# graphdeco-inria/reduced-3dgs

Measured on AMD Instinct MI355X. Metric: train iters/s (fwd+bwd) + Mpix/s render, 500k Gaussians @1600x1062, higher is better.
Workload: dtype f32

## Files before the change

reduced-3dgs_amd/csrc/binning.hip:

```cpp
#include <cstdlib>
#include <cstring>
#include <mutex>
#include <string>

#include <rocprim/rocprim.hpp>

#include "depth_sort.h"

namespace r3 {

struct GatherTiles {
    const uint32_t* tiles;
    __host__ __device__ uint32_t operator()(uint32_t id) const { return tiles[id]; }
};

size_t depth_sort_temp_bytes(size_t P)
{
    size_t a = 0, b = 0;
    uint32_t* n = nullptr;
    R3_HIP(rocprim::radix_sort_pairs(nullptr, a, n, n, rocprim::counting_iterator<uint32_t>(0), n, P, 0, 32));
    auto it = rocprim::make_transform_iterator(n, GatherTiles{n});
    R3_HIP(rocprim::inclusive_scan(nullptr, b, it, n, P, rocprim::plus<uint32_t>()));
    return (a > b ? a : b) + 256;
}

void run_generic_depth_sort(int P, GeomState& g, hipStream_t s)
{
    size_t bytes = g.temp_bytes;
    R3_HIP(rocprim::radix_sort_pairs(g.temp, bytes, g.depth_key, g.key_sorted, rocprim::counting_iterator<uint32_t>(0),
                                     g.order, (size_t)P, 0, 32, s));
    bytes = g.temp_bytes;
    auto it = rocprim::make_transform_iterator(g.order, GatherTiles{g.tiles});
    R3_HIP(rocprim::inclusive_scan(g.temp, bytes, it, g.offsets, (size_t)P, rocprim::plus<uint32_t>(), s));
}

__global__ __launch_bounds__(1024) void header_reduce_kernel(const HeaderArgs* __restrict__ ap)
{
    __shared__ uint32_t s_red[16][6];
    const HeaderArgs a = *ap;
    const PrePartial all = reduce_partials(a.parts, a.n_parts, s_red);
    if (threadIdx.x == 0) write_header(a, all);
}

void issue_header_reduce(const HeaderArgs* a, hipStream_t s)
{
    hipLaunchKernelGGL(header_reduce_kernel, dim3(1), dim3(1024), 0, s, a);
}

PairLayout pair_layout(int P, size_t n_tiles)
{
    static const int forced = [] {
        const char* v = getenv("R3DGS_TILE_SORT");
        return !v ? 0 : std::string(v) == "wide" ? 1 : std::string(v) == "split" ? 2 : 0;
    }();
    PairLayout l;
    l.tile_bits = (int)higher_msb((uint32_t)n_tiles);
    const int rb = (int)higher_msb((uint32_t)P);
    const bool fits16 = n_tiles <= 65536;
    if (forced == 1 || (forced == 2 && !fits16))
        l.wide = 1;
    else if (forced == 2)
        l.wide = 2;
    else
        l.wide = l.tile_bits + rb > 32 ? (fits16 ? 2 : 1) : 0;
// ... 94 lines not shown
        }
        if (lane == 0) {
            s_j[w] = j;
            if (w == 0) s_start0 = j == 0 ? 0u : offsets[j - 1];
        }
    }
    __syncthreads();
    const uint32_t j_lo = s_j[0], j_hi = s_j[1];
    const uint32_t n = min(j_hi - j_lo + 1u, (uint32_t)kEmitSlice);
    const uint32_t start0 = s_start0;
    auto stage = [&](uint32_t r0, uint32_t nr) {
        for (uint32_t k = threadIdx.x; k < nr; k += 256) {
            const uint32_t g = j_lo + r0 + k, id = a.order[g];
            s_start[k] = r0 + k == 0 ? start0 : offsets[g - 1];
            s_id[k] = id;
            s_rect[k] = a.rect_sorted ? a.rect_sorted[g] : a.rect[id];
        }
    };
    const uint32_t nr0 = min(n, (uint32_t)kEmitStage);
    stage(0u, nr0);
    __syncthreads();
    for (uint32_t k = threadIdx.x; k < n; k += 256) {
        const uint32_t start = k < nr0 ? s_start[k] : offsets[j_lo + k - 1];
        a.rec[k < nr0 ? s_id[k] : a.order[j_lo + k]].pair_start = start;
        if (start >= pos0) s_owner[start - pos0] = (unsigned short)k;
    }
    __syncthreads();
    {
        constexpr int E = kEmitPerBlock / 256;
        const int lane = threadIdx.x & 63, w = threadIdx.x >> 6;
        uint32_t v[E];
#pragma unroll
        for (int i = 0; i < E; i++) v[i] = s_owner[threadIdx.x * E + i];
#pragma unroll
        for (int i = 1; i < E; i++) v[i] = max(v[i], v[i - 1]);
        uint32_t incl = v[E - 1];
        for (int off = 1; off < 64; off <<= 1) {
            const uint32_t up = (uint32_t)__shfl_up((int)incl, off);
            if (lane >= off) incl = max(incl, up);
        }
        if (lane == 63) s_wmax[w] = incl;
        uint32_t before = (uint32_t)__shfl_up((int)incl, 1);
        if (lane == 0) before = 0;
        __syncthreads();
        for (int q = 0; q < w; q++) before = max(before, s_wmax[q]);
#pragma unroll
        for (int i = 0; i < E; i++) s_owner[threadIdx.x * E + i] = (unsigned short)max(v[i], before);
    }
    typedef typename IO::Reg Word;
    const int rank_bits = a.rank_bits;
    for (uint32_t r0 = 0; r0 < n; r0 += (uint32_t)kEmitStage) {
        const uint32_t nr = min(n - r0, (uint32_t)kEmitStage);
        __syncthreads();
        if (r0 > 0) {
            stage(r0, nr);
            __syncthreads();
        }
#pragma unroll
        for (int e = 0; e < kEmitPerBlock / 256; e++) {
            const uint32_t pos = pos0 + threadIdx.x + (uint32_t)e * 256u;
            if (pos < pos1) {
                const uint32_t lo = (uint32_t)s_owner[pos - pos0] - r0;
                if (lo < nr) {
                    const uint32_t local = pos - s_start[lo];
                    const ushort4 r = s_rect[lo];
                    const uint32_t w = (uint32_t)r.z - (uint32_t)r.x;
                    const uint32_t ty = local / w, tx = local - ty * w;
                    const uint32_t tile = ((uint32_t)r.y + ty) * (uint32_t)a.gx + (uint32_t)r.x + tx;
                    IO::store(a.words_out, nullptr, a.cap, pos, ((Word)tile << rank_bits) | (Word)s_id[lo]);
                    if (a.pair_rank) a.pair_rank[pos] = s_id[lo];
                    atomicAdd(&s_hist[tile & (uint32_t)(bins - 1)], 1u);
                }
            }
        }
    }
    __syncthreads();
    if ((int)threadIdx.x < bins) a.radix_rows[(size_t)threadIdx.x * a.row_stride + blk] = s_hist[threadIdx.x];
}

template <class IO>
__global__ __launch_bounds__(256) void emit_pairs_kernel(const EmitArgs* __restrict__ ap)
{
    const EmitArgs a = *ap;
    const uint32_t R = a.hdr->num_pairs;
    for (uint32_t t = blockIdx.x * 256u + threadIdx.x; t < a.n_tiles; t += gridDim.x * 256u) a.ranges[t] = make_uint2(0u, 0u);
    for (uint32_t blk = blockIdx.x; blk * (uint32_t)kEmitPerBlock < R; blk += gridDim.x) {
        emit_pairs_block<IO>(a, R, blk);
        __syncthreads();
    }
}

template <class IO>
__device__ __forceinline__ void radix_hist_block(const RadixArgs& a, uint32_t R, uint32_t blk)
// ... 300 lines not shown
```

reduced-3dgs_amd/csrc/blend.hip:

```cpp
#include <cstdlib>

#include "blend_math.h"
#include "common.h"

namespace r3 {

constexpr int kChunk = 64;

#if defined(R3_TIMELINE) || defined(R3_TIMELINE_FWD)
__device__ unsigned long long g_timeline[4 * 65536];
#define R3_TL_BEGIN_(id) const unsigned long long tl0_ = __builtin_amdgcn_s_memtime(); const uint32_t tlid_ = (id);
#define R3_TL_END_(extra)                                                                                                \
    if (threadIdx.x == 0 && tlid_ < 65536u) {                                                                            \
        g_timeline[4 * tlid_] = tl0_;                                                                                     \
        g_timeline[4 * tlid_ + 1] = __builtin_amdgcn_s_memtime();                                                         \
        g_timeline[4 * tlid_ + 2] = (unsigned long long)__builtin_amdgcn_s_getreg((4 << 0) | (0 << 6) | (31 << 11)) |     \
                                    ((unsigned long long)__builtin_amdgcn_s_getreg((20 << 0) | (0 << 6) | (31 << 11)) << 32); \
        g_timeline[4 * tlid_ + 3] = (unsigned long long)(extra);                                                          \
    }
#endif
#if defined(R3_TIMELINE)
#define R3_TL_BEGIN(id) R3_TL_BEGIN_(id)
#define R3_TL_END(extra) R3_TL_END_(extra)
#else
// ... 525 lines not shown
                }
            if (hit != 0ull) {
                const float z = wave_reduce9(sg, lane);
                int joff = j * kGradStride;
                asm("" : "+s"(joff));
                if (writer) s_grad_slot[joff] = z;
                contributed |= 1ull << j;
#ifndef R3_OLD_TRIP_FORMS
                {
                    typedef float v4f __attribute__((ext_vector_type(4)));
                    const volatile v4f __attribute__((address_space(3)))* zp =
                        (const volatile v4f __attribute__((address_space(3)))*)reinterpret_cast<float*>(s_zero);
                    const v4f z0 = zp[0], z1 = zp[1];
                    const float z2 = *(const volatile float __attribute__((address_space(3)))*)(zp + 2);
                    sg.sx = z0.x; sg.sy = z0.y; sg.sxx = z0.z; sg.sxy = z0.w;
                    sg.syy = z1.x; sg.sm = z1.y; sg.r = z1.z; sg.g = z1.w; sg.b = z2;
                }
#else
                sg.sx = sg.sy = sg.sxx = sg.sxy = sg.syy = sg.sm = sg.r = sg.g = sg.b = 0.f;
#endif
            }
        }
        __syncthreads();
        if (lane < n && ((contributed >> lane) & 1ull)) {
            const float4 c = s_rec[lane].c;
            const uint32_t rect_min = __float_as_uint(c.y), width = __float_as_uint(c.z) & 0xffffu;
            const uint32_t slot = __float_as_uint(c.w) + ((uint32_t)tile_y - (rect_min >> 16)) * width +
                                  ((uint32_t)tile_x - (rect_min & 0xffffu));
            float4* dst = reinterpret_cast<float4*>(a.pair_grad + (size_t)slot * kPairStride);
            const float* src = s_grad + lane * kGradStride;
            SplatSums u;
            u.sx = src[0];
            u.sy = src[1];
            u.sxx = src[2];
            u.sxy = src[3];
            u.syy = src[4];
            u.sm = src[5];
            u.r = src[6];
            u.g = src[7];
            u.b = src[8];
            const SplatGrad g = splat_grad_of(load_splat(s_rec[lane]), u);
            dst[0] = make_float4(g.mx * half_w, g.my * half_h, g.cA, g.cB);
            dst[1] = make_float4(g.cC, g.op, g.r, g.g);
            dst[2] = make_float4(g.b, 0.f, 0.f, 0.f);
            if (kPairStride >= 16) dst[3] = make_float4(0.f, 0.f, 0.f, 0.f);
            a.pair_flag[slot] = 1;
        }
    }
    R3_TL_END(hi - lo)
}

#if defined(R3_TIMELINE) || defined(R3_TIMELINE_FWD)
extern "C" int r3dgs_debug_timeline(unsigned long long* host, int n)
{
    return (int)hipMemcpyFromSymbol(host, HIP_SYMBOL(g_timeline), sizeof(unsigned long long) * 4 * (size_t)n);
}
#endif

constexpr int kOrderThreads = 1024, kOrderClasses = 1024;

__device__ __forceinline__ uint32_t unit_segments(uint32_t list_len, uint32_t deepest, uint32_t thr, uint32_t walk)
{
    if (list_len < thr || deepest <= (1u << walk)) return 1u;
    return min((deepest + (1u << walk) - 1u) >> walk, (uint32_t)kBwdSegMax);
}
__device__ __forceinline__ uint32_t unit_weight(const uint4& d, uint32_t s, uint32_t n, uint32_t walk)
{
    if (n == 1u) return d.x + d.y + d.z + d.w;
    const uint32_t lo = s << walk, hi = s + 1u < n ? lo + (1u << walk) : 0xFFFFFFFFu;
    auto part = [&](uint32_t q) { return min(max(q, lo), hi) - lo; };
    return part(d.x) + part(d.y) + part(d.z) + part(d.w);
}

template <int KEEP>
__global__ __launch_bounds__(kOrderThreads) void unit_order_kernel(BwdPassArgs* dst, BwdPassArgs v)
{
    __shared__ uint32_t s_count[kOrderClasses];
    __shared__ uint32_t s_scan[kOrderThreads / 64];
    constexpr int kWalks = 4;
    __shared__ uint32_t s_max;
    const uint32_t tid = threadIdx.x, lane_id = tid & 63u;
    if (blockIdx.x == 0) install_block_from_kernarg(dst, (int)tid, kOrderThreads);
    const uint32_t list = blockIdx.x, all_tiles = v.blend.nblocks;
    const TileGrid grid{(uint32_t)v.blend.gx, all_tiles / (uint32_t)v.blend.gx};
    const uint4* __restrict__ qd = reinterpret_cast<const uint4*>(v.blend.quad_depth);
    const uint2* __restrict__ ranges = v.blend.ranges;
    const uint32_t cap = v.blend.units_cap / kOrderLists;
    uint32_t* __restrict__ order = v.blend.tile_order + list * cap;
    uint32_t* __restrict__ trailer = v.blend.tile_order + v.blend.units_cap + 2u * list;
    const uint32_t n_tiles = grid.list_slots(list);
    auto tile_of = [&](uint32_t j) { return grid.list_tile(list, j); };
    const uint32_t seg_log2 = (v.blend.segments != 0 && v.blend.ckpt != nullptr && all_tiles <= (1u << kUnitTileBits))
                                  ? v.blend.hdr->ckpt : 0u;
    const uint32_t thr = seg_log2 ? v.blend.hdr->ckpt_thr : 0xFFFFFFFFu;
    const uint32_t fit = bwd_list_fit(v.blend.hdr->num_pairs, grid);
    s_count[tid] = 0u;
    if (tid == 0) s_max = 0u;
    __syncthreads();
    const bool keep = n_tiles <= (uint32_t)(KEEP * kOrderThreads);
    uint4 w[KEEP];
    uint32_t len[KEEP], tl[KEEP];
    auto load = [&](uint32_t t, uint4& d, uint32_t& l) {
        d = make_uint4(0u, 0u, 0u, 0u);
        l = 0u;
        const uint32_t tile = t < n_tiles ? tile_of(t) : 0xFFFFFFFFu;
// ... 160 lines not shown
        for (uint32_t t0 = 0; t0 < n_tiles; t0 += kOrderThreads) {
            uint4 d;
            uint32_t l;
            load(t0 + tid, d, l);
            const uint32_t n = d.x + d.y + d.z + d.w == 0u ? 0u
                               : (walk ? unit_segments(l, max(max(d.x, d.y), max(d.z, d.w)), thr, walk) : 1u);
            uint32_t f = 0u;
            if (n > 1u) {
                f = min(min(d.x, d.y), min(d.z, d.w)) >> walk;
                f = min(f, n == (uint32_t)kBwdSegMax ? n - 1u : n);
            }
            place(t0 + tid < n_tiles ? tile_of(t0 + tid) : 0u, d, n, f, full_base(f), 0u, false);
        }
    }
}

template <bool REUSE>
static void launch_bwd(uint32_t nblocks, uint32_t units_cap, BwdPassArgs* dst, const BwdPassArgs& v, hipStream_t s)
{
    if (v.blend.tile_order) {
        static const int lds_pad = env_int("R3DGS_BWD_LDS_PAD", 0, 0, 65536);
        hipLaunchKernelGGL((blend_bwd_kernel<4, REUSE, false>), dim3(units_cap), dim3(64), lds_pad, s, dst, v);
    } else {
        hipLaunchKernelGGL((blend_bwd_kernel<4, REUSE, true>), dim3(nblocks), dim3(64), 0, s, dst, v);
    }
}

void issue_unit_order(const BwdPlan& p, BwdPassArgs* dst, const BwdPassArgs& v, hipStream_t s)
{
    if (!v.blend.tile_order) return;
    const uint32_t slots = TileGrid{(uint32_t)p.gx, (uint32_t)p.gy}.list_slots(0);
    if (slots <= (uint32_t)kOrderThreads)
        hipLaunchKernelGGL(unit_order_kernel<1>, dim3(kOrderLists), dim3(kOrderThreads), 0, s, dst, v);
    else if (slots <= 2u * (uint32_t)kOrderThreads)
        hipLaunchKernelGGL(unit_order_kernel<2>, dim3(kOrderLists), dim3(kOrderThreads), 0, s, dst, v);
    else
        hipLaunchKernelGGL(unit_order_kernel<8>, dim3(kOrderLists), dim3(kOrderThreads), 0, s, dst, v);
}

void issue_blend_backward(const BwdPlan& p, BwdPassArgs* dst, const BwdPassArgs& v, hipStream_t s)
{
    const uint32_t nblocks = (uint32_t)(p.gx * p.gy);
    if (v.blend.quad_masks)
        launch_bwd<true>(nblocks, p.units_cap, dst, v, s);
    else
        launch_bwd<false>(nblocks, p.units_cap, dst, v, s);
}

}
```

reduced-3dgs_amd/csrc/capi.hip:

```cpp
#include "../../include/r3dgs_rasterizer.h"
#include "../../include/r3dgs_quantised.h"

#include <time.h>

#include <atomic>
#include <random>
#include <chrono>
#include <cmath>
#include <cstddef>
#include <cstdlib>
#include <cstring>
#include <deque>
#include <map>
#include <mutex>
#include <unordered_map>
#include <vector>

#include "common.h"
#include "quant_math.h"

namespace r3 {
int env_int(const char* env, int dflt, int lo, int hi)
{
    const char* v = getenv(env);
// ... 632 lines not shown
    d.offsets = g.offsets;
    uint32_t* const block_first = (b && fuse_header && !p.generic_depth_sort) ? b->block_first : nullptr;
    d.block_first = block_first;
    d.block_cap = p.reserve / (uint32_t)kRadixBlock + 2u;

    const PairLayout& l = p.layout;
    const size_t Tn = (size_t)p.gx * p.gy;
    if (b) {
        const uint32_t stride = radix_row_stride(p.reserve);
        EmitArgs& e = a.emit;
        e.P = c.P;
        e.gx = p.gx;
        e.hdr = g.header;
        e.order = g.order;
        e.offsets = g.offsets;
        e.block_first = block_first;
        e.rect = g.rect;
        e.rect_sorted = p.generic_depth_sort ? nullptr : g.rect_sorted;
        e.rec = g.rec;
        e.rank_bits = l.rank_bits;
        e.digit_bits = l.digit_bits;
        e.words_out = b->words_a;
        e.cap = p.reserve;
        e.pair_rank = l.wide == 1 ? b->pair_rank : nullptr;
        e.ranges = img.ranges;
        e.n_tiles = (uint32_t)Tn;
        e.radix_rows = b->radix_rows;
        e.row_stride = stride;
        const char* src = b->words_a;
        for (int k = 0; k < l.passes; k++) {
            char* dst = l.wide ? ((k & 1) ? b->words_a : b->words_b) : ((k & 1) ? b->words_c : b->words_b);
            RadixArgs& r = a.radix[k];
            r.hdr = g.header;
            r.in = src;
            r.out = dst;
            r.ids_out = (l.wide == 2 && k == l.passes - 1) ? b->point_list : nullptr;
            r.cap = p.reserve;
            r.shift = l.rank_bits + k * l.digit_bits;
            r.digit_bits = l.digit_bits;
            r.rank_bits = l.rank_bits;
            r.tile_shift = k * l.digit_bits;
            r.rows = b->radix_rows;
            r.base = b->radix_base;
            r.total = b->radix_total + k * kMaxRadixBins;
            r.row_stride = stride;
            src = dst;
        }
// ... 507 lines not shown
        bb.rec = geom.rec;
        bb.final_T = img.final_T;
        bb.n_contrib = img.n_contrib;
        bb.dL_dpix = dL_dpix;
        bb.W = width;
        bb.H = height;
        bb.gx = plan.gx;
        bb.nblocks = (uint32_t)(plan.gx * plan.gy * (4 / plan.bwd_ppl));
        bb.bg = background;
        bb.pair_grad = bin.pair_grad;
        bb.pair_flag = bin.pair_flag;
        bb.quad_masks = binning_buffer && keep_quad_masks() ? bin.quad_masks : nullptr;
        bb.tile_order = (heaviest_tiles_first() && plan.has_pairs && (size_t)plan.gx * plan.gy <= ((size_t)1 << kUnitTileBits))
                            ? bin.unit_order : nullptr;
        bb.units_cap = plan.units_cap;
        bb.quad_depth = img.quad_depth;
        bb.ckpt = plan.has_pairs ? bin.ckpt : nullptr;
        bb.hdr = geom.header;
        bb.segments = bwd_segments();
        PairReduceArgs& pr = a.reduce;
        pr.hdr = geom.header;
        pr.pair_grad = bin.pair_grad;
        pr.pair_flag = bin.pair_flag;
        pr.pair_rank = bin.pair_rank;
        pr.rank_mask = plan.layout.wide ? 0xFFFFFFFFu : (1u << plan.layout.rank_bits) - 1u;
        pr.order = nullptr;
        pr.rec = geom.rec;
        pr.tiles = geom.tiles;
        pr.acc = geom.acc;
        pr.wave_part = bin.wave_part;
        {
            static std::atomic<unsigned long long> stamp{[] {
                std::random_device rd;
                return ((unsigned long long)rd() << 32) ^ (unsigned long long)rd() ^ 0x9E3779B97F4A7C15ull;
            }()};
            const unsigned long long st = stamp.fetch_add(1);
            pr.stamp0 = (uint32_t)st;
            pr.stamp1 = (uint32_t)(st >> 32);
        }
        PreBwdArgs& pb = a.pre;
        FwdInputs& in = pb.in;
        in.P = P;
        in.M = M;
        in.degrees = D;
        in.means3D = means3D;
        in.scales = scales;
        in.rotations = rotations;
        in.opacities = nullptr;
        in.shs = colors_precomp ? nullptr : shs;
        in.cov3D_precomp = cov3D_precomp;
        in.colors_precomp = colors_precomp;
        ViewParams& view = pb.view;
        view.view = viewmatrix;
        view.proj = projmatrix;
        view.campos = campos;
        view.bg = background;
        view.tan_fovx = tan_fovx;
        view.tan_fovy = tan_fovy;
        view.W = width;
        view.H = height;
        view.scale_modifier = scale_modifier;
        pb.radii = radii;
// ... 352 lines not shown
```

reduced-3dgs_amd/csrc/common.h:

```cpp
#pragma once
#include <hip/hip_runtime.h>
#include <stddef.h>
#include <stdint.h>

#include <functional>
#include <stdexcept>
#include <string>

#include "gauss_math.h"
#include "param_math.h"

namespace r3 {

constexpr size_t kAlign = 256;
constexpr int kPairGrad = 9;
constexpr int kPieceStride = 9;
constexpr int kAccStride = 12;
constexpr int kPairStride = 12;
static_assert(kAccStride >= 12 && kAccStride % 4 == 0 && kPairStride >= 12 && kPairStride % 4 == 0,
              "the kernels move three float4 per row");

constexpr int kPreBlockSize = 256;
struct PrePartial {
    uint32_t visible;
    uint32_t num_rendered;
    uint32_t depth_max;
    uint32_t depth_inv_min;
    uint32_t binned;
    uint32_t rendered_ref;
    uint32_t pad[2];
};
static_assert(sizeof(PrePartial) == 32, "two 16-byte loads per partial");
struct GeomHeader {
    uint32_t visible, num_rendered, depth_max, depth_inv_min;
    uint32_t num_pairs;
    uint32_t reserve;
    uint32_t sort_overflow;
    uint32_t binned;
    uint32_t rendered_ref;
    uint32_t sh_cache;
    uint32_t ckpt;
    uint32_t ckpt_thr;
    uint32_t pad[52];
};
static_assert(sizeof(GeomHeader) == 256, "header = 256 B");
inline size_t pre_partials(size_t P) { return (P + kPreBlockSize - 1) / kPreBlockSize; }

struct PassInfo {
    uint32_t seq;
    uint32_t num_rendered;
    uint32_t visible;
    uint32_t reserve;
    uint32_t sort_overflow;
// ... 161 lines not shown
        const uint32_t tx = k % bx * kListBlock + o % kListBlock, ty = k / bx * kListBlock + o / kListBlock;
        return tx < gx && ty < gy ? ty * gx + tx : 0xFFFFFFFFu;
    }
    R3_HD uint32_t list_tiles_max() const
    {
        const size_t m = (size_t)((blocks() + kOrderLists - 1) / kOrderLists) * kListBlockTiles;
        return (uint32_t)(m < n() ? m : n());
    }
};
R3_HD uint32_t bwd_list_fit(uint32_t pairs, const TileGrid& g)
{
    const size_t extra = (size_t)pairs >> kBwdSegMinLog2, most = 8 * g.n();
    return g.list_tiles_max() + (uint32_t)((extra < most ? extra : most) / kOrderLists);
}
inline uint32_t bwd_units_cap(uint32_t reserve, const TileGrid& g) { return (bwd_list_fit(reserve, g) + 1u) * kOrderLists; }
int bwd_segment_log2();
int bwd_segment_factor_pct();

struct BinState {
    uint32_t* point_list;
    float* pair_grad;
    float* wave_part;
    unsigned char* pair_flag;
    uint32_t* pair_rank;
    char* words_a;
    char* words_b;
    char* words_c;
    uint32_t* radix_rows;
    uint32_t* radix_base;
    uint32_t* radix_total;
    uint32_t* block_first;
    unsigned long long* quad_masks;
    uint32_t* unit_order;
    float4* ckpt;
    char* end;
    static BinState carve(char* base, size_t R, int wide, const TileGrid& grid)
    {
        const size_t Tn = grid.n();
        Carver c(base);
        BinState b;
        b.point_list = c.take<uint32_t>(R);
        b.pair_grad = c.take<float>(R * kPairStride);
        b.wave_part = c.take<float>((R / 64 + 1) * 2 * kPieceStride);
        b.pair_flag = c.take<unsigned char>(R);
        if (wide == 1) {
            b.pair_rank = c.take<uint32_t>(R);
            b.words_a = reinterpret_cast<char*>(c.take<unsigned long long>(R));
            b.words_b = reinterpret_cast<char*>(c.take<unsigned long long>(R));
            b.words_c = nullptr;
        } else if (wide == 2) {
            b.words_a = reinterpret_cast<char*>(c.take<unsigned long long>(R));
            b.words_b = reinterpret_cast<char*>(c.take<unsigned long long>(R));
            b.words_c = nullptr;
            b.pair_rank = reinterpret_cast<uint32_t*>(b.words_a);
        } else {
            b.words_a = reinterpret_cast<char*>(c.take<uint32_t>(R));
            b.words_b = reinterpret_cast<char*>(c.take<uint32_t>(R));
            b.words_c = reinterpret_cast<char*>(c.take<uint32_t>(R));
            b.pair_rank = reinterpret_cast<uint32_t*>(b.words_a);
        }
        b.radix_rows = c.take<uint32_t>((size_t)kMaxRadixBins * radix_row_stride(R));
        b.radix_base = c.take<uint32_t>((size_t)kMaxRadixBins * radix_row_stride(R));
        b.radix_total = c.take<uint32_t>(kMaxRadixPasses * kMaxRadixBins);
        b.quad_masks = c.take<unsigned long long>((R / 64 + Tn + 2) * 4);
        b.block_first = c.take<uint32_t>(R / kRadixBlock + 2);
        b.unit_order = c.take<uint32_t>((size_t)bwd_units_cap((uint32_t)R, grid) + 2 * kOrderLists);
        b.ckpt = c.take<float4>(ckpt_slots(R, Tn) * 256);
        b.end = c.p;
        return b;
    }
};

R3_HD size_t quad_mask_slot(uint32_t first, uint32_t chunk, uint32_t tile)
{
    return (size_t)(first >> 6) + chunk + tile;
}

struct ImageState {
    float* final_T;
    uint32_t* n_contrib;
    uint2* ranges;
    uint32_t* quad_depth;
// ... 127 lines not shown
    float* dL_dcolor;
    float* dL_dmean3D;
    float* dL_dcov3D;
    float* dL_dsh;
    float* dL_dscale;
    float* dL_drot;
    float* dL_dconic;
};

struct PreArgs {
    FwdInputs in;
    ViewParams view;
    GRec* rec;
    ushort4* rect;
    uint32_t* depth_key;
    uint32_t* tiles;
    PrePartial* partials;
    int* radii;
    int color_blocks;
    int tight;
    float* sh_ddir;
};
struct HeaderArgs {
    const PrePartial* parts;
    int n_parts;
    GeomHeader* hdr;
    PassInfo* info;
    uint32_t ticket;
    uint32_t reserve;
    uint32_t stamp_sort;
    uint32_t sh_cache;
    uint32_t ckpt;
    uint32_t ckpt_factor_pct, n_tiles;
};
struct DepthArgs {
    int P, nb, rows, per_block;
    int fuse_header;
    const uint32_t* key;
    const uint32_t* tiles;
    GeomHeader* hdr;
    PassInfo* info;
    uint32_t ticket;
    DepthSortScratch* ds;
    unsigned long long* hist_rows;
    uint32_t* hist_base;
    uint32_t* key_sorted;
    uint32_t* bucket_id;
// ... 70 lines not shown
    const uint2* ranges;
    const uint32_t* point_list;
    const GRec* rec;
    const float* final_T;
    const uint32_t* n_contrib;
    const float* dL_dpix;
    int W, H, gx;
    uint32_t nblocks;
    const float* bg;
    float* pair_grad;
    unsigned char* pair_flag;
    const unsigned long long* quad_masks;
    uint32_t* tile_order;
    uint32_t units_cap;
    const uint32_t* quad_depth;
    const float4* ckpt;
    const GeomHeader* hdr;
    int segments;
};
struct PairReduceArgs {
    const GeomHeader* hdr;
    const float* pair_grad;
    unsigned char* pair_flag;
    const uint32_t* pair_rank;
    uint32_t rank_mask;
    const uint32_t* order;
    const GRec* rec;
    const uint32_t* tiles;
    float* acc;
    float* wave_part;
    uint32_t stamp0, stamp1;
};
struct PreBwdArgs {
    FwdInputs in;
    ViewParams view;
    const int* radii;
    const GRec* rec;
    const uint32_t* tiles;
    const float* acc;
    const float* wave_part;
    uint32_t stamp0, stamp1;
    const GeomHeader* header;
    float lambda_sh;
    const float* sh_ddir;
    int stagger;
    BwdOutputs out;
    const float* shs_rest;
    float* dL_dsh_rest;
};

struct FwdPassArgs {
    PreArgs pre;
    HeaderArgs header;
    DepthArgs depth;
    EmitArgs emit;
    RadixArgs radix[kMaxRadixPasses];
    RangesArgs ranges;
    BlendFwdArgs blend;
    const float* shs_rest;
    QuantInputs quant;
};
struct BwdPassArgs {
    BlendBwdArgs blend;
    PairReduceArgs reduce;
    PreBwdArgs pre;
};
static_assert(sizeof(FwdPassArgs) <= 3072 && sizeof(BwdPassArgs) <= 3072, "pass blocks travel as by-value kernel arguments");

struct FwdPlan {
    int P, M, W, H, gx, gy;
    uint32_t reserve;
    uint32_t grid_pairs;
    PairLayout layout;
    int nb;
    int ragged, counters;
    int color_grid;
    int color_split[3];
    int generic_depth_sort;
    int tight;
    int raw_params;
    int quant;
};
struct BwdPlan {
    int P, M, W, H, gx, gy;
    uint32_t reserve, grid_pairs;
    uint32_t units_cap;
    PairLayout layout;
    int bwd_ppl;
// ... 56 lines not shown
```

reduced-3dgs_amd/csrc/depth_sort.h:

```cpp
#pragma once
#include "common.h"

namespace r3 {

template <class T>
__device__ inline T block256_inclusive_scan(T v, T* s_w)
{
    const int lane = threadIdx.x & 63, w = threadIdx.x >> 6;
    for (int off = 1; off < 64; off <<= 1) {
        const T up = __shfl_up(v, off);
        if (lane >= off) v += up;
    }
    __syncthreads();
    if (lane == 63) s_w[w] = v;
    __syncthreads();
    T add = 0;
    for (int k = 0; k < w; k++) add += s_w[k];
    return v + add;
}

template <int BITS>
__device__ __forceinline__ unsigned long long match_digit(uint32_t d, bool valid)
{
    unsigned long long peers = __ballot(valid);
// ... 32 lines not shown
};
__device__ inline DepthRange make_depth_range(uint32_t mx, uint32_t mi, int nb)
{
    DepthRange r;
    const uint32_t kmax = mx, kmin = ~mi;
    r.kmin = kmin;
    r.nb = nb;
    r.scale = kmax >= kmin ? (float)nb / ((float)(kmax - kmin) + 1.0f) : 0.0f;
    return r;
}
__device__ inline int depth_bucket(uint32_t key, const DepthRange& r)
{
    if (key == 0xFFFFFFFFu) return r.nb;
    const int b = (int)((float)(key - r.kmin) * r.scale);
    return min(max(b, 0), r.nb - 1);
}

inline size_t depth_hist_lds(int nb) { return (size_t)(nb + 1) * sizeof(unsigned long long); }
inline size_t depth_scatter_lds(int nb) { return (size_t)2 * (nb + 2) * sizeof(uint32_t) + 256 * sizeof(unsigned long long); }
constexpr size_t kBucketSortLds = (size_t)kBucketCap * 8 + 256 * 4 + (256 + 256 + 4 * 256 + 4) * 4;

__device__ inline PrePartial reduce_partials(const PrePartial* __restrict__ parts, int n, uint32_t (*s_red)[6])
{
    PrePartial acc = {0u, 0u, 0u, 0u, 0u, 0u, {0u, 0u}};
    for (int i = threadIdx.x; i < n; i += blockDim.x) {
        const uint4 v = reinterpret_cast<const uint4*>(parts)[2 * i], w = reinterpret_cast<const uint4*>(parts)[2 * i + 1];
        acc.visible += v.x;
        acc.num_rendered += v.y;
        acc.depth_max = max(acc.depth_max, v.z);
        acc.depth_inv_min = max(acc.depth_inv_min, v.w);
        acc.binned += w.x;
        acc.rendered_ref += w.y;
    }
    for (int off = 32; off > 0; off >>= 1) {
        acc.visible += (uint32_t)__shfl_xor((int)acc.visible, off);
        acc.num_rendered += (uint32_t)__shfl_xor((int)acc.num_rendered, off);
        acc.depth_max = max(acc.depth_max, (uint32_t)__shfl_xor((int)acc.depth_max, off));
        acc.depth_inv_min = max(acc.depth_inv_min, (uint32_t)__shfl_xor((int)acc.depth_inv_min, off));
        acc.binned += (uint32_t)__shfl_xor((int)acc.binned, off);
        acc.rendered_ref += (uint32_t)__shfl_xor((int)acc.rendered_ref, off);
    }
    const int w = threadIdx.x >> 6, nw = (blockDim.x + 63) >> 6;
    if ((threadIdx.x & 63) == 0) {
        s_red[w][0] = acc.visible;
        s_red[w][1] = acc.num_rendered;
        s_red[w][2] = acc.depth_max;
        s_red[w][3] = acc.depth_inv_min;
        s_red[w][4] = acc.binned;
        s_red[w][5] = acc.rendered_ref;
    }
    __syncthreads();
    PrePartial out = {0u, 0u, 0u, 0u, 0u, 0u, {0u, 0u}};
    for (int k = 0; k < nw; k++) {
        out.visible += s_red[k][0];
        out.num_rendered += s_red[k][1];
        out.depth_max = max(out.depth_max, s_red[k][2]);
        out.depth_inv_min = max(out.depth_inv_min, s_red[k][3]);
        out.binned += s_red[k][4];
        out.rendered_ref += s_red[k][5];
    }
    __syncthreads();
    return out;
}

__device__ inline void write_header(const HeaderArgs& a, const PrePartial& all)
{
    GeomHeader* hdr = a.hdr;
    hdr->visible = all.visible;
    hdr->num_rendered = all.num_rendered;
    hdr->depth_max = all.depth_max;
    hdr->depth_inv_min = all.depth_inv_min;
    hdr->num_pairs = min(all.num_rendered, a.reserve);
    hdr->reserve = a.reserve;
    hdr->sort_overflow = 0u;
    hdr->binned = all.binned;
    hdr->rendered_ref = all.rendered_ref;
    hdr->sh_cache = a.sh_cache;
    hdr->ckpt = a.ckpt;
    {
        const unsigned long long mean_pct = (unsigned long long)hdr->num_pairs * a.ckpt_factor_pct / (a.n_tiles ? a.n_tiles : 1u);
        const uint32_t thr = (uint32_t)min(mean_pct / 100ull, 0x7FFFFFFFull);
        hdr->ckpt_thr = a.ckpt ? max(thr, 2u << a.ckpt) : 0xFFFFFFFFu;
    }
    volatile PassInfo* info = a.info;
    if (info) {
        info->num_rendered = all.rendered_ref;
        info->pairs = all.num_rendered;
        info->visible = all.visible;
        info->reserve = a.reserve;
        info->sort_overflow = 0u;
        __threadfence_system();
        if (a.stamp_sort) info->sort_seq = a.ticket;
        info->seq = a.ticket;
    }
}

__device__ inline void depth_hist_role(const DepthArgs& a, const HeaderArgs& h, char* smem, int wg)
{
    __shared__ uint32_t s_red[16][6];
    unsigned long long* hist = reinterpret_cast<unsigned long long*>(smem);
    const int P = a.P, nb = a.nb;
    for (int b = threadIdx.x; b <= nb; b += 256) hist[b] = 0;
    uint32_t dmax, dinv;
    if (wg == 0 && threadIdx.x == 0) a.ds->big_count = 0u;
    if (a.fuse_header) {
        const PrePartial all = reduce_partials(h.parts, h.n_parts, s_red);
        if (wg == 0 && threadIdx.x == 0) write_header(h, all);
        dmax = all.depth_max;
        dinv = all.depth_inv_min;
    } else {
        dmax = a.hdr->depth_max;
        dinv = a.hdr->depth_inv_min;
    }
    const DepthRange rng = make_depth_range(dmax, dinv, nb);
    __syncthreads();
    for (int base = wg * a.per_block; base < min(P, (wg + 1) * a.per_block); base += kHistBatch) {
        uint32_t kv[kHistPerThread], tv[kHistPerThread];
#pragma unroll
        for (int k = 0; k < kHistPerThread; k++) {
            const int i = base + k * 256 + threadIdx.x;
            kv[k] = i < P ? a.key[i] : 0xFFFFFFFFu;
            tv[k] = i < P ? a.tiles[i] : 0u;
        }
#pragma unroll
        for (int k = 0; k < kHistPerThread; k++)
            if (base + k * 256 + (int)threadIdx.x < P)
                atomicAdd(&hist[depth_bucket(kv[k], rng)], ((unsigned long long)tv[k] << kCountBits) | 1ull);
    }
    __syncthreads();
    unsigned long long* row = a.hist_rows + (size_t)wg * (nb + 1);
// ... 606 lines not shown
```

reduced-3dgs_amd/csrc/preprocess.hip:

```cpp
#include <cstdlib>
#include <map>
#include <mutex>

#include "depth_sort.h"
#include "quant_math.h"

namespace r3 {

constexpr int kPreBlock = kPreBlockSize;
constexpr int kMaxCoeff = 16;
constexpr int kRowFloats = 3 * kMaxCoeff;
constexpr int kWaveShFloats = 64 * kRowFloats + (64 * kRowFloats) / 32;

template <bool ROWS48>
__device__ __forceinline__ int skew(int e)
{
    if (ROWS48) return e + (int)(((uint32_t)e * 43691u) >> 21);
    return e + (e >> 5);
}

template <bool ROWS48>
struct ShRowLds {
    const float* base;
    int roff;
// ... 184 lines not shown
    }
    const unsigned long long vmask = __ballot(o.radius > 0);
    const bool binned = o.tiles > 0;
    const unsigned long long bmask = __ballot(binned);
    uint32_t tsum = o.tiles, rsum = o.tiles_ref;
    uint32_t dmax = binned ? __float_as_uint(o.depth) : 0u, dinv = binned ? ~__float_as_uint(o.depth) : 0u;
    for (int off = 32; off > 0; off >>= 1) {
        tsum += (uint32_t)__shfl_xor((int)tsum, off);
        rsum += (uint32_t)__shfl_xor((int)rsum, off);
        dmax = max(dmax, (uint32_t)__shfl_xor((int)dmax, off));
        dinv = max(dinv, (uint32_t)__shfl_xor((int)dinv, off));
    }
    __shared__ uint32_t s_cnt[kPreBlock / 64][6];
    if (lane == 0) {
        s_cnt[wave][0] = (uint32_t)__popcll(vmask);
        s_cnt[wave][1] = tsum;
        s_cnt[wave][2] = dmax;
        s_cnt[wave][3] = dinv;
        s_cnt[wave][4] = (uint32_t)__popcll(bmask);
        s_cnt[wave][5] = rsum;
    }
    __syncthreads();
    if (tid == 0) {
        PrePartial pp = {0u, 0u, 0u, 0u, 0u, 0u, {0u, 0u}};
        for (int k = 0; k < kPreBlock / 64; k++) {
            pp.visible += s_cnt[k][0];
            pp.num_rendered += s_cnt[k][1];
            pp.depth_max = max(pp.depth_max, s_cnt[k][2]);
            pp.depth_inv_min = max(pp.depth_inv_min, s_cnt[k][3]);
            pp.binned += s_cnt[k][4];
            pp.rendered_ref += s_cnt[k][5];
        }
        a.partials[blockIdx.x] = pp;
    }
}

constexpr size_t kColorLds = sizeof(float) * (kPreBlock / 64) * kWaveShFloats;

__device__ __forceinline__ void store_color(GRec* r, const float* rgb, uint32_t cbits)
{
    r->r = rgb[0];
    r->g = rgb[1];
    r->b = rgb[2];
    if (cbits) r->width_clamp |= cbits << 16;
}

template <bool RAGGED, int BLOCK, bool SPLIT = false>
// ... 436 lines not shown
```

reduced-3dgs_amd/csrc/preprocess_bwd.hip:

```cpp
#include "common.h"

namespace r3 {

constexpr int kBwdBlock = 64;
constexpr int kBwdWaveShFloats = 64 * 48 + (64 * 48) / 32;

template <bool ROWS48>
__device__ __forceinline__ int bskew(int e)
{
    if (ROWS48) return e + (int)(((uint32_t)e * 43691u) >> 21);
    return e + (e >> 5);
}

template <bool ROWS48>
struct ShRowLdsRW {
    float* base;
    int roff;
    __device__ __forceinline__ float at(int e) const { return ROWS48 ? base[e] : base[bskew<false>(roff + e)]; }
    __device__ __forceinline__ void put(int e, float v) const
    {
        if (ROWS48)
            base[e] = v;
        else
            base[bskew<false>(roff + e)] = v;
// ... 73 lines not shown
                                                  float (&v)[kPairGrad], uint32_t key_before, uint32_t key_after)
{
#define R3_SEG_STEP(CTRL, RMASK)                                                                                          \
    {                                                                                                                     \
        const uint32_t ku = (uint32_t)__builtin_amdgcn_update_dpp((int)~key, (int)key, CTRL, RMASK, 0xf, false);          \
        const bool take = ku == key;                                                                                      \
        _Pragma("unroll") for (int k = 0; k < kPairGrad; k++)                                                             \
        {                                                                                                                 \
            const float vu = __builtin_bit_cast(                                                                          \
                float, __builtin_amdgcn_update_dpp(0, __builtin_bit_cast(int, v[k]), CTRL, RMASK, 0xf, false));           \
            if (take) v[k] += vu;                                                                                         \
        }                                                                                                                 \
    }
    R3_SEG_STEP(0x111, 0xf)
    R3_SEG_STEP(0x112, 0xf)
    R3_SEG_STEP(0x114, 0xf)
    R3_SEG_STEP(0x118, 0xf)
    R3_SEG_STEP(0x142, 0xa)
    R3_SEG_STEP(0x143, 0xc)
#undef R3_SEG_STEP
    const uint32_t knext = (uint32_t)__shfl_down((int)key, 1);
    const uint32_t key0 = (uint32_t)__builtin_amdgcn_readfirstlane((int)key);
    if (valid && (lane == 63 || knext != key)) {
        const uint32_t gid = a.order ? global_ptr(a.order)[key] : key;
        const bool from_before = key == key0 && key_before == key;
        const bool into_next = lane == 63 && key_after == key;
        if (!from_before && !into_next) {
            auto* dst = reinterpret_cast<R3_GLOBAL float4*>(global_ptr(a.acc) + (size_t)gid * kAccStride);
            bool nz = false;
#pragma unroll
            for (int k = 0; k < kPairGrad; k++) nz |= v[k] != 0.f;
            if (nz) {
                dst[0] = make_float4(v[0], v[1], v[2], v[3]);
                dst[1] = make_float4(v[4], v[5], v[6], v[7]);
                dst[2] = make_float4(v[8], __uint_as_float(a.stamp0), __uint_as_float(a.stamp1), 0.f);
            }
        } else {
            R3_GLOBAL float* wp = global_ptr(a.wave_part) + (size_t)(e >> 6) * 2 * kPieceStride;
            if (from_before) {
#pragma unroll
                for (int k = 0; k < kPairGrad; k++) wp[k] = v[k];
            }
            if (into_next) {
#pragma unroll
                for (int k = 0; k < kPairGrad; k++) wp[kPieceStride + k] = v[k];
            }
        }
    }
}

__global__ __launch_bounds__(256) void pair_reduce_kernel(const PairReduceArgs* __restrict__ ap)
{
    const PairReduceArgs a = *ap;
    const uint32_t R = global_ptr(a.hdr)->num_pairs;
    constexpr uint32_t kPerBlock = 256u * kReduceGroups;
  for (uint32_t blk = blockIdx.x; blk * kPerBlock < R; blk += gridDim.x) {
    const R3_GLOBAL float* __restrict__ pair_grad = global_ptr(a.pair_grad);
    R3_GLOBAL unsigned char* __restrict__ pair_flag = global_ptr(a.pair_flag);
    const R3_GLOBAL uint32_t* __restrict__ pair_gid = global_ptr(a.pair_rank);
    const uint32_t rank_mask = a.rank_mask;
    const int lane = threadIdx.x & 63, wave = threadIdx.x >> 6;
    const uint32_t e0 = blk * kPerBlock + (uint32_t)wave * (64u * kReduceGroups) + (uint32_t)lane;
    float v[kReduceGroups][kPairGrad];
    uint32_t key[kReduceGroups], kb[kReduceGroups], ka[kReduceGroups];
    bool flag[kReduceGroups];
#pragma unroll
    for (int g = 0; g < kReduceGroups; g++) {
        const uint32_t e = e0 + 64u * g, gbase = e & ~63u;
        key[g] = e < R ? pair_gid[e] & rank_mask : 0xFFFFFFFFu;
        flag[g] = e < R && pair_flag[e] != 0;
        kb[g] = gbase > 0u && gbase < R ? pair_gid[gbase - 1u] & rank_mask : 0xFFFFFFFFu;
        ka[g] = gbase + 64u < R ? pair_gid[gbase + 64u] & rank_mask : 0xFFFFFFFFu;
    }
#pragma unroll
    for (int g = 0; g < kReduceGroups; g++) {
        const uint32_t e = e0 + 64u * g;
#pragma unroll
        for (int k = 0; k < kPairGrad; k++) v[g][k] = 0.f;
        if (flag[g]) {
            pair_flag[e] = 0;
            const auto* src = reinterpret_cast<const R3_GLOBAL float4*>(pair_grad + (size_t)e * kPairStride);
            const float4 r0 = src[0], r1 = src[1];
            v[g][0] = r0.x; v[g][1] = r0.y; v[g][2] = r0.z; v[g][3] = r0.w;
            v[g][4] = r1.x; v[g][5] = r1.y; v[g][6] = r1.z; v[g][7] = r1.w;
            v[g][8] = src[2].x;
        }
    }
#pragma unroll
    for (int g = 0; g < kReduceGroups; g++) {
        const uint32_t e = e0 + 64u * g;
        pair_reduce_group(a, e, lane, e < R, key[g], v[g], kb[g], ka[g]);
    }
  }
}

// ... 313 lines not shown
```

Baseline: 1580.

## Assign pair gradient slots by Gaussian index via a slab-scan instead of depth order

Per-Gaussian pair slots are now laid out in Gaussian-index order: a per-block base is computed by scanning the preprocess partials, and a new slab role (fused into the unit-order kernel, or launched alone) writes pair_start and a slot-to-Gaussian map. The emit kernel no longer writes pair_start or pair_rank, and the pair reduce reads the Gaussian id directly without an order indirection. This is meant to remove scattered writes in emit and the indirect lookup in reduce, and to make the gradient stores and accumulation more contiguous. In exchange it adds a scan in the header kernel, extra blocks in the unit-order launch, and truncation handling through a binary search plus a depth-key comparison.

Result: slower. 1562 (-1.1%).

```diff
diff --git a/reduced-3dgs_amd/csrc/binning.hip b/reduced-3dgs_amd/csrc/binning.hip
--- a/reduced-3dgs_amd/csrc/binning.hip
+++ b/reduced-3dgs_amd/csrc/binning.hip
@@ -40,6 +40,7 @@
     const HeaderArgs a = *ap;
     const PrePartial all = reduce_partials(a.parts, a.n_parts, s_red);
     if (threadIdx.x == 0) write_header(a, all);
+    scan_pair_base(a.parts, a.n_parts, &s_red[0][0]);
 }
 
 void issue_header_reduce(const HeaderArgs* a, hipStream_t s)
@@ -180,7 +181,6 @@
     __syncthreads();
     for (uint32_t k = threadIdx.x; k < n; k += 256) {
         const uint32_t start = k < nr0 ? s_start[k] : offsets[j_lo + k - 1];
-        a.rec[k < nr0 ? s_id[k] : a.order[j_lo + k]].pair_start = start;
         if (start >= pos0) s_owner[start - pos0] = (unsigned short)k;
     }
     __syncthreads();
@@ -226,7 +226,6 @@
                     const uint32_t ty = local / w, tx = local - ty * w;
                     const uint32_t tile = ((uint32_t)r.y + ty) * (uint32_t)a.gx + (uint32_t)r.x + tx;
                     IO::store(a.words_out, nullptr, a.cap, pos, ((Word)tile << rank_bits) | (Word)s_id[lo]);
-                    if (a.pair_rank) a.pair_rank[pos] = s_id[lo];
                     atomicAdd(&s_hist[tile & (uint32_t)(bins - 1)], 1u);
                 }
             }
diff --git a/reduced-3dgs_amd/csrc/blend.hip b/reduced-3dgs_amd/csrc/blend.hip
--- a/reduced-3dgs_amd/csrc/blend.hip
+++ b/reduced-3dgs_amd/csrc/blend.hip
@@ -571,7 +571,7 @@
             }
         }
         __syncthreads();
-        if (lane < n && ((contributed >> lane) & 1ull)) {
+        if (lane < n && ((contributed >> lane) & 1ull) && __float_as_uint(s_rec[lane].c.w) != 0xFFFFFFFFu) {
             const float4 c = s_rec[lane].c;
             const uint32_t rect_min = __float_as_uint(c.y), width = __float_as_uint(c.z) & 0xffffu;
             const uint32_t slot = __float_as_uint(c.w) + ((uint32_t)tile_y - (rect_min >> 16)) * width +
@@ -608,6 +608,79 @@
 
 constexpr int kOrderThreads = 1024, kOrderClasses = 1024;
 
+constexpr uint32_t kSlabBlock = kOrderThreads;
+static_assert(kSlabBlock % kPreBlockSize == 0, "a block of the slab role starts at a preprocess workgroup's first Gaussian");
+inline uint32_t slab_role_groups(int P)
+{
+    const uint32_t blocks = ((uint32_t)P + kSlabBlock - 1u) / kSlabBlock;
+    return blocks < 496u ? blocks : 496u;
+}
+__device__ __forceinline__ void slab_slots_role(const PairReduceArgs& r, const SlabArgs& x, uint32_t wg, uint32_t n_wg,
+                                                uint32_t* s_excl, uint32_t* s_w)
+{
+    const uint32_t tid = threadIdx.x, lane = tid & 63u, w = tid >> 6;
+    const uint32_t P = r.P, R = r.hdr->num_pairs;
+    const bool truncated = r.hdr->num_rendered > R;
+    uint32_t cut_key = 0u, cut_id = 0u;
+    if (truncated) {
+        uint32_t lo = 0u, hi = P;
+        while (lo < hi) {
+            const uint32_t mid = (lo + hi) >> 1;
+            if (x.offsets[mid] > R) hi = mid; else lo = mid + 1u;
+        }
+        cut_id = x.order[min(lo, P - 1u)];
+        cut_key = x.depth_key[cut_id];
+    }
+    const uint32_t* __restrict__ tiles = r.tiles;
+    uint32_t* __restrict__ slot_gid = r.slot_gid;
+    for (uint32_t blk = wg; blk * kSlabBlock < P; blk += n_wg) {
+        const uint32_t i = blk * kSlabBlock + tid;
+        const uint32_t t = i < P ? tiles[i] : 0u;
+        const uint32_t base = r.partials[blk * (kSlabBlock / (uint32_t)kPreBlockSize)].pair_base;
+        uint32_t dkey = 0u;
+        if (truncated && t > 0u) dkey = x.depth_key[i];
+        uint32_t incl = t;
+        for (int off = 1; off < 64; off <<= 1) {
+            const uint32_t up = (uint32_t)__shfl_up((int)incl, off);
+            if (lane >= (uint32_t)off) incl += up;
+        }
+        if (lane == 63u) s_w[w] = incl;
+        __syncthreads();
+        uint32_t before = 0u, total = 0u;
+        for (uint32_t k = 0; k < kSlabBlock / 64u; k++) {
+            const uint32_t c = s_w[k];
+            if (k < w) before += c;
+            total += c;
+        }
+        const uint32_t excl = before + incl - t;
+        s_excl[tid] = excl;
+        if (t > 0u) {
+            const uint32_t S = base + excl;
+            bool keeps = S < R && t <= R - S;
+            if (truncated) keeps = keeps && (dkey < cut_key || (dkey == cut_key && i < cut_id));
+            r.rec[i].pair_start = keeps ? S : 0xFFFFFFFFu;
+        }
+        __syncthreads();
+        const uint32_t n = base < R ? min(total, R - base) : 0u;
+        for (uint32_t e = tid; e < n; e += kSlabBlock) {
+            uint32_t lo = 0u;
+#pragma unroll
+            for (uint32_t step = kSlabBlock / 2u; step > 0u; step >>= 1)
+                if (s_excl[lo + step] <= e) lo += step;
+            slot_gid[base + e] = blk * kSlabBlock + lo;
+        }
+        __syncthreads();
+    }
+}
+
+__global__ __launch_bounds__(kOrderThreads) void slab_slots_kernel(BwdPassArgs* dst, BwdPassArgs v)
+{
+    __shared__ uint32_t s_excl[kSlabBlock];
+    __shared__ uint32_t s_w[kSlabBlock / 64];
+    if (blockIdx.x == 0) install_block_from_kernarg(dst, (int)threadIdx.x, kOrderThreads);
+    slab_slots_role(v.reduce, v.slab, blockIdx.x, gridDim.x, s_excl, s_w);
+}
+
 __device__ __forceinline__ uint32_t unit_segments(uint32_t list_len, uint32_t deepest, uint32_t thr, uint32_t walk)
 {
     if (list_len < thr || deepest <= (1u << walk)) return 1u;
@@ -630,6 +703,10 @@
     __shared__ uint32_t s_max;
     const uint32_t tid = threadIdx.x, lane_id = tid & 63u;
     if (blockIdx.x == 0) install_block_from_kernarg(dst, (int)tid, kOrderThreads);
+    if (blockIdx.x >= kOrderLists) {
+        slab_slots_role(v.reduce, v.slab, blockIdx.x - kOrderLists, gridDim.x - kOrderLists, s_count, s_scan);
+        return;
+    }
     const uint32_t list = blockIdx.x, all_tiles = v.blend.nblocks;
     const TileGrid grid{(uint32_t)v.blend.gx, all_tiles / (uint32_t)v.blend.gx};
     const uint4* __restrict__ qd = reinterpret_cast<const uint4*>(v.blend.quad_depth);
@@ -836,20 +913,25 @@
         static const int lds_pad = env_int("R3DGS_BWD_LDS_PAD", 0, 0, 65536);
         hipLaunchKernelGGL((blend_bwd_kernel<4, REUSE, false>), dim3(units_cap), dim3(64), lds_pad, s, dst, v);
     } else {
-        hipLaunchKernelGGL((blend_bwd_kernel<4, REUSE, true>), dim3(nblocks), dim3(64), 0, s, dst, v);
+        hipLaunchKernelGGL((blend_bwd_kernel<4, REUSE, false>), dim3(nblocks), dim3(64), 0, s, dst, v);
     }
 }
 
 void issue_unit_order(const BwdPlan& p, BwdPassArgs* dst, const BwdPassArgs& v, hipStream_t s)
 {
-    if (!v.blend.tile_order) return;
+    const uint32_t role = slab_role_groups(p.P);
+    if (!v.blend.tile_order) {
+        hipLaunchKernelGGL(slab_slots_kernel, dim3(role), dim3(kOrderThreads), 0, s, dst, v);
+        return;
+    }
     const uint32_t slots = TileGrid{(uint32_t)p.gx, (uint32_t)p.gy}.list_slots(0);
+    const dim3 grid(kOrderLists + role);
     if (slots <= (uint32_t)kOrderThreads)
-        hipLaunchKernelGGL(unit_order_kernel<1>, dim3(kOrderLists), dim3(kOrderThreads), 0, s, dst, v);
+        hipLaunchKernelGGL(unit_order_kernel<1>, grid, dim3(kOrderThreads), 0, s, dst, v);
     else if (slots <= 2u * (uint32_t)kOrderThreads)
-        hipLaunchKernelGGL(unit_order_kernel<2>, dim3(kOrderLists), dim3(kOrderThreads), 0, s, dst, v);
+        hipLaunchKernelGGL(unit_order_kernel<2>, grid, dim3(kOrderThreads), 0, s, dst, v);
     else
-        hipLaunchKernelGGL(unit_order_kernel<8>, dim3(kOrderLists), dim3(kOrderThreads), 0, s, dst, v);
+        hipLaunchKernelGGL(unit_order_kernel<8>, grid, dim3(kOrderThreads), 0, s, dst, v);
 }
 
 void issue_blend_backward(const BwdPlan& p, BwdPassArgs* dst, const BwdPassArgs& v, hipStream_t s)
diff --git a/reduced-3dgs_amd/csrc/capi.hip b/reduced-3dgs_amd/csrc/capi.hip
--- a/reduced-3dgs_amd/csrc/capi.hip
+++ b/reduced-3dgs_amd/csrc/capi.hip
@@ -678,7 +678,7 @@
         e.digit_bits = l.digit_bits;
         e.words_out = b->words_a;
         e.cap = p.reserve;
-        e.pair_rank = l.wide == 1 ? b->pair_rank : nullptr;
+        e.pair_rank = nullptr;
         e.ranges = img.ranges;
         e.n_tiles = (uint32_t)Tn;
         e.radix_rows = b->radix_rows;
@@ -1232,9 +1232,9 @@
         pr.hdr = geom.header;
         pr.pair_grad = bin.pair_grad;
         pr.pair_flag = bin.pair_flag;
-        pr.pair_rank = bin.pair_rank;
-        pr.rank_mask = plan.layout.wide ? 0xFFFFFFFFu : (1u << plan.layout.rank_bits) - 1u;
-        pr.order = nullptr;
+        pr.slot_gid = bin.slot_gid;
+        pr.P = (uint32_t)P;
+        pr.partials = geom.partials;
         pr.rec = geom.rec;
         pr.tiles = geom.tiles;
         pr.acc = geom.acc;
@@ -1248,6 +1248,9 @@
             pr.stamp0 = (uint32_t)st;
             pr.stamp1 = (uint32_t)(st >> 32);
         }
+        a.slab.offsets = geom.offsets;
+        a.slab.order = geom.order;
+        a.slab.depth_key = geom.depth_key;
         PreBwdArgs& pb = a.pre;
         FwdInputs& in = pb.in;
         in.P = P;
diff --git a/reduced-3dgs_amd/csrc/common.h b/reduced-3dgs_amd/csrc/common.h
--- a/reduced-3dgs_amd/csrc/common.h
+++ b/reduced-3dgs_amd/csrc/common.h
@@ -28,7 +28,8 @@
     uint32_t depth_inv_min;
     uint32_t binned;
     uint32_t rendered_ref;
-    uint32_t pad[2];
+    uint32_t pair_base;
+    uint32_t pad;
 };
 static_assert(sizeof(PrePartial) == 32, "two 16-byte loads per partial");
 struct GeomHeader {
@@ -236,7 +237,7 @@
     float* pair_grad;
     float* wave_part;
     unsigned char* pair_flag;
-    uint32_t* pair_rank;
+    uint32_t* slot_gid;
     char* words_a;
     char* words_b;
     char* words_c;
@@ -258,7 +259,7 @@
         b.wave_part = c.take<float>((R / 64 + 1) * 2 * kPieceStride);
         b.pair_flag = c.take<unsigned char>(R);
         if (wide == 1) {
-            b.pair_rank = c.take<uint32_t>(R);
+            b.slot_gid = c.take<uint32_t>(R);
             b.words_a = reinterpret_cast<char*>(c.take<unsigned long long>(R));
             b.words_b = reinterpret_cast<char*>(c.take<unsigned long long>(R));
             b.words_c = nullptr;
@@ -266,12 +267,12 @@
             b.words_a = reinterpret_cast<char*>(c.take<unsigned long long>(R));
             b.words_b = reinterpret_cast<char*>(c.take<unsigned long long>(R));
             b.words_c = nullptr;
-            b.pair_rank = reinterpret_cast<uint32_t*>(b.words_a);
+            b.slot_gid = reinterpret_cast<uint32_t*>(b.words_a);
         } else {
             b.words_a = reinterpret_cast<char*>(c.take<uint32_t>(R));
             b.words_b = reinterpret_cast<char*>(c.take<uint32_t>(R));
             b.words_c = reinterpret_cast<char*>(c.take<uint32_t>(R));
-            b.pair_rank = reinterpret_cast<uint32_t*>(b.words_a);
+            b.slot_gid = reinterpret_cast<uint32_t*>(b.words_a);
         }
         b.radix_rows = c.take<uint32_t>((size_t)kMaxRadixBins * radix_row_stride(R));
         b.radix_base = c.take<uint32_t>((size_t)kMaxRadixBins * radix_row_stride(R));
@@ -445,7 +446,7 @@
     float* sh_ddir;
 };
 struct HeaderArgs {
-    const PrePartial* parts;
+    PrePartial* parts;
     int n_parts;
     GeomHeader* hdr;
     PassInfo* info;
@@ -562,10 +563,10 @@
     const GeomHeader* hdr;
     const float* pair_grad;
     unsigned char* pair_flag;
-    const uint32_t* pair_rank;
-    uint32_t rank_mask;
-    const uint32_t* order;
-    const GRec* rec;
+    uint32_t* slot_gid;
+    uint32_t P;
+    const PrePartial* partials;
+    GRec* rec;
     const uint32_t* tiles;
     float* acc;
     float* wave_part;
@@ -600,10 +601,16 @@
     const float* shs_rest;
     QuantInputs quant;
 };
+struct SlabArgs {
+    const uint32_t* offsets;
+    const uint32_t* order;
+    const uint32_t* depth_key;
+};
 struct BwdPassArgs {
     BlendBwdArgs blend;
     PairReduceArgs reduce;
     PreBwdArgs pre;
+    SlabArgs slab;
 };
 static_assert(sizeof(FwdPassArgs) <= 3072 && sizeof(BwdPassArgs) <= 3072, "pass blocks travel as by-value kernel arguments");
 
diff --git a/reduced-3dgs_amd/csrc/depth_sort.h b/reduced-3dgs_amd/csrc/depth_sort.h
--- a/reduced-3dgs_amd/csrc/depth_sort.h
+++ b/reduced-3dgs_amd/csrc/depth_sort.h
@@ -78,7 +78,7 @@
 
 __device__ inline PrePartial reduce_partials(const PrePartial* __restrict__ parts, int n, uint32_t (*s_red)[6])
 {
-    PrePartial acc = {0u, 0u, 0u, 0u, 0u, 0u, {0u, 0u}};
+    PrePartial acc = {0u, 0u, 0u, 0u, 0u, 0u, 0u, 0u};
     for (int i = threadIdx.x; i < n; i += blockDim.x) {
         const uint4 v = reinterpret_cast<const uint4*>(parts)[2 * i], w = reinterpret_cast<const uint4*>(parts)[2 * i + 1];
         acc.visible += v.x;
@@ -106,7 +106,7 @@
         s_red[w][5] = acc.rendered_ref;
     }
     __syncthreads();
-    PrePartial out = {0u, 0u, 0u, 0u, 0u, 0u, {0u, 0u}};
+    PrePartial out = {0u, 0u, 0u, 0u, 0u, 0u, 0u, 0u};
     for (int k = 0; k < nw; k++) {
         out.visible += s_red[k][0];
         out.num_rendered += s_red[k][1];
@@ -117,6 +117,28 @@
     }
     __syncthreads();
     return out;
+}
+
+__device__ inline void scan_pair_base(PrePartial* __restrict__ parts, int n, uint32_t* s_w)
+{
+    const int nt = (int)blockDim.x, per = (n + nt - 1) / nt, b0 = (int)threadIdx.x * per;
+    const int lane = threadIdx.x & 63, w = threadIdx.x >> 6;
+    uint32_t sum = 0u;
+    for (int k = b0; k < min(n, b0 + per); k++) sum += parts[k].num_rendered;
+    uint32_t incl = sum;
+    for (int off = 1; off < 64; off <<= 1) {
+        const uint32_t up = (uint32_t)__shfl_up((int)incl, off);
+        if (lane >= off) incl += up;
+    }
+    __syncthreads();
+    if (lane == 63) s_w[w] = incl;
+    __syncthreads();
+    uint32_t run = incl - sum;
+    for (int k = 0; k < w; k++) run += s_w[k];
+    for (int k = b0; k < min(n, b0 + per); k++) {
+        parts[k].pair_base = run;
+        run += parts[k].num_rendered;
+    }
 }
 
 __device__ inline void write_header(const HeaderArgs& a, const PrePartial& all)
@@ -162,6 +184,7 @@
     if (a.fuse_header) {
         const PrePartial all = reduce_partials(h.parts, h.n_parts, s_red);
         if (wg == 0 && threadIdx.x == 0) write_header(h, all);
+        if (wg == a.rows - 1) scan_pair_base(h.parts, h.n_parts, &s_red[0][0]);
         dmax = all.depth_max;
         dinv = all.depth_inv_min;
     } else {
diff --git a/reduced-3dgs_amd/csrc/preprocess.hip b/reduced-3dgs_amd/csrc/preprocess.hip
--- a/reduced-3dgs_amd/csrc/preprocess.hip
+++ b/reduced-3dgs_amd/csrc/preprocess.hip
@@ -230,7 +230,7 @@
     }
     __syncthreads();
     if (tid == 0) {
-        PrePartial pp = {0u, 0u, 0u, 0u, 0u, 0u, {0u, 0u}};
+        PrePartial pp = {0u, 0u, 0u, 0u, 0u, 0u, 0u, 0u};
         for (int k = 0; k < kPreBlock / 64; k++) {
             pp.visible += s_cnt[k][0];
             pp.num_rendered += s_cnt[k][1];
diff --git a/reduced-3dgs_amd/csrc/preprocess_bwd.hip b/reduced-3dgs_amd/csrc/preprocess_bwd.hip
--- a/reduced-3dgs_amd/csrc/preprocess_bwd.hip
+++ b/reduced-3dgs_amd/csrc/preprocess_bwd.hip
@@ -119,7 +119,7 @@
     const uint32_t knext = (uint32_t)__shfl_down((int)key, 1);
     const uint32_t key0 = (uint32_t)__builtin_amdgcn_readfirstlane((int)key);
     if (valid && (lane == 63 || knext != key)) {
-        const uint32_t gid = a.order ? global_ptr(a.order)[key] : key;
+        const uint32_t gid = key;
         const bool from_before = key == key0 && key_before == key;
         const bool into_next = lane == 63 && key_after == key;
         if (!from_before && !into_next) {
@@ -154,8 +154,7 @@
   for (uint32_t blk = blockIdx.x; blk * kPerBlock < R; blk += gridDim.x) {
     const R3_GLOBAL float* __restrict__ pair_grad = global_ptr(a.pair_grad);
     R3_GLOBAL unsigned char* __restrict__ pair_flag = global_ptr(a.pair_flag);
-    const R3_GLOBAL uint32_t* __restrict__ pair_gid = global_ptr(a.pair_rank);
-    const uint32_t rank_mask = a.rank_mask;
+    const R3_GLOBAL uint32_t* __restrict__ pair_gid = global_ptr(a.slot_gid);
     const int lane = threadIdx.x & 63, wave = threadIdx.x >> 6;
     const uint32_t e0 = blk * kPerBlock + (uint32_t)wave * (64u * kReduceGroups) + (uint32_t)lane;
     float v[kReduceGroups][kPairGrad];
@@ -164,10 +163,10 @@
 #pragma unroll
     for (int g = 0; g < kReduceGroups; g++) {
         const uint32_t e = e0 + 64u * g, gbase = e & ~63u;
-        key[g] = e < R ? pair_gid[e] & rank_mask : 0xFFFFFFFFu;
+        key[g] = e < R ? pair_gid[e] : 0xFFFFFFFFu;
         flag[g] = e < R && pair_flag[e] != 0;
-        kb[g] = gbase > 0u && gbase < R ? pair_gid[gbase - 1u] & rank_mask : 0xFFFFFFFFu;
-        ka[g] = gbase + 64u < R ? pair_gid[gbase + 64u] & rank_mask : 0xFFFFFFFFu;
+        kb[g] = gbase > 0u && gbase < R ? pair_gid[gbase - 1u] : 0xFFFFFFFFu;
+        ka[g] = gbase + 64u < R ? pair_gid[gbase + 64u] : 0xFFFFFFFFu;
     }
 #pragma unroll
     for (int g = 0; g < kReduceGroups; g++) {
```
